# YihanWangAstro/VegasAfterglow

Hardware: AMD Instinct MI355X
Metric: light-curves/sec (single model) and MCMC walker-steps/sec at 1/2/4/8 MI355X (higher is better)
Workload: dtype f64

## Files before the change

vegasafterglow_amd/csrc/vag_capi.hip:

```cpp
#include <hip/hip_runtime.h>

#include <algorithm>
#include <cmath>
#include <cstdarg>
#include <cstdio>
#include <cstdlib>
#include <cstring>
#include <memory>
#include <string>
#include <vector>
#include <atomic>
#include <chrono>
#include <condition_variable>
#include <map>
#include <mutex>
#include <shared_mutex>

#include "vag_ic_kernels.h"
#include "vag_kernels.h"
#include "vag_rs_kernels.h"
#include "vag_fit_rows.h"
#include "vag_grid_rows.h"
#include "vag_sky.h"
#include "vag_debug_math.h"
// ... 537 lines not shown
}

}

static int ctx_init(vag_ctx* c) {
    HIPCHK(hipStreamCreateWithFlags(&c->own_stream, hipStreamNonBlocking));
    c->stream = c->own_stream;
    for (auto& e : c->ev) HIPCHK(hipEventCreate(&e));
    HIPCHK(hipEventCreateWithFlags(&c->ev_handoff, hipEventDisableTiming));
    HIPCHK(hipDeviceGetAttribute(&c->n_cus, hipDeviceAttributeMultiprocessorCount, c->device));
    for (const void* fn : {reinterpret_cast<const void*>(vag_flux_grid_kernel<false, FLUX_SYN>),
                           reinterpret_cast<const void*>(vag_flux_grid_kernel<true, FLUX_SYN>),
                           reinterpret_cast<const void*>(vag_flux_grid_kernel<false, FLUX_SYN_IC>),
                           reinterpret_cast<const void*>(vag_flux_grid_kernel<false, FLUX_SSC>),
                           reinterpret_cast<const void*>(vag_flux_grid_kernel<false, FLUX_SYN, false, 256>),
                           reinterpret_cast<const void*>(vag_flux_grid_kernel<false, FLUX_SYN_IC, false, 256>),
                           reinterpret_cast<const void*>(vag_flux_grid_kernel<false, FLUX_SSC, false, 256>),
                           reinterpret_cast<const void*>(vag_flux_grid_kernel<false, FLUX_SYN, true>),
                           reinterpret_cast<const void*>(vag_flux_grid_kernel<false, FLUX_SYN_IC, true>),
                           reinterpret_cast<const void*>(vag_flux_grid_kernel<false, FLUX_SSC, true>),
                           reinterpret_cast<const void*>(vag_flux_grid_kernel<false, FLUX_FUSED>),
                           reinterpret_cast<const void*>(vag_flux_grid_kernel<false, FLUX_FUSED, false, 256>),
                           reinterpret_cast<const void*>(vag_flux_grid_kernel<false, FLUX_FUSED, true>),
                           reinterpret_cast<const void*>(vag_flux_series_kernel<FLUX_SYN, true>),
                           reinterpret_cast<const void*>(vag_flux_series_kernel<FLUX_SYN_IC, true>),
                           reinterpret_cast<const void*>(vag_flux_series_kernel<FLUX_SSC, true>)})
        HIPCHK(hipFuncSetAttribute(fn, hipFuncAttributeMaxDynamicSharedMemorySize, 160 * 1024));
    {
        std::vector<double> lut(2 * KN_LUT_N);
        const double step = (KN_LG2_XMAX - KN_LG2_XMIN) / (double)(KN_LUT_N - 1);
        for (int i = 0; i < KN_LUT_N; ++i) {
            const double x = std::exp2(KN_LG2_XMIN + step * (double)i);
            double ratio;
            if (x < 1e-2) {
                ratio = 1 - 2 * x;
            } else if (x > 1e2) {
                ratio = 3. / 8 * (std::log(2 * x) + 0.5) / x;
            } else {
                const double l = std::log1p(2.0 * x), invx = 1.0 / x, invx2 = invx * invx;
                const double invt1 = 1.0 / (1.0 + 2.0 * x), invt1_2 = invt1 * invt1;
                ratio = 0.75 * ((1.0 + x) * invx2 * invx * (2.0 * x * (1.0 + x) * invt1 - l) + 0.5 * l * invx -
                                (1.0 + 3.0 * x) * invt1_2);
            }
            lut[i] = ratio;
            lut[KN_LUT_N + i] = std::log2(ratio);
        }
// ... 551 lines not shown
    long long lo = 4;
    if (c->total_pairs / 16 >= 2048) lo = 16;
    if (c->total_pairs / 64 >= 4096) lo = 64;
    ppb = std::max(ppb, lo);
    ppb = std::min<long long>(ppb, std::max(1, c->max_pairs));
    return (int)std::max<long long>(1, ppb);
}

static int flux_ks(const vag_ctx* c) {
    int cap = 512;
    if (const char* e = vag_hook("VAG_FLUX_K_CAP")) cap = std::max(4, std::atoi(e));
    return std::max(2, std::min(c->max_k, cap));
}

static int* work_counters(vag_ctx* c) { return reinterpret_cast<int*>(reinterpret_cast<char*>(c->d_plan.p) + sizeof(VagDevPlan)) + 4; }

static size_t flux_grid_lds_bytes(int mode, int ks, int nt, int nnu) {
    const size_t slots = (size_t)nt * nnu;
    size_t d = (size_t)(VAG_NPAR + 4) * ks + (size_t)ks * nnu + 2 * (size_t)nt + nnu + SP_LDS_DOUBLES + slots;
    if (mode == FLUX_FUSED) d += 6 * (size_t)ks + (size_t)ks * nnu + slots;
    return sizeof(double) * d + sizeof(int) * nt + 16;
}

int run_flux_series(vag_ctx* c, const vag_model_params* d_params, int nb, const double* d_lg2t, const double* d_lg2nu, int n,
                    double* d_out, int mode = FLUX_SYN, int n_bands = 0, int grid_nt = 0);

static void launch_reduce(hipStream_t st, const vag_model_params* d_params, const VagGridMeta* meta, const double* partial, int max_blocks,
                          int ppb, int nt, int nnu, const double* d_bandw, double* d_out, int nb,
                          int* work_counter = nullptr ) {
    if (d_bandw) {
        hipLaunchKernelGGL(vag_reduce_kernel, dim3((nt + 255) / 256, nb), dim3(256), 0, st, d_params, meta, partial, max_blocks, ppb, nt, nnu,
                           d_bandw, d_out, work_counter);
    } else {
        const int slots = nt * nnu;
        hipLaunchKernelGGL(vag_reduce_grid_kernel, dim3((slots + REDUCE_SLOTS - 1) / REDUCE_SLOTS, nb), dim3(REDUCE_GROUPS * REDUCE_SLOTS), 0, st,
                           d_params, meta, partial, max_blocks, ppb, slots, d_out, work_counter);
    }
}

constexpr int FLUX_PERSIST_MIN_PPB = 128;
template <bool COUNT, int MODE, bool SPREAD = false, int THREADS = FLUX_THREADS, bool PIECES = false>
static bool launch_flux_grid(vag_ctx* c, FluxArgs a, int nb, size_t lds, int persist) {
    const auto fn = vag_flux_grid_kernel<COUNT, MODE, SPREAD, THREADS, PIECES, true>;
    int wg = -1;
    if (persist) {
        for (const auto& e : c->flux_occ)
            if (e.fn == reinterpret_cast<const void*>(fn) && e.lds == lds) wg = e.wg;
        if (wg < 0) {
            (void)hipFuncSetAttribute(reinterpret_cast<const void*>(fn), hipFuncAttributeMaxDynamicSharedMemorySize, 160 * 1024);
            if (hipOccupancyMaxActiveBlocksPerMultiprocessor(&wg, fn, THREADS, lds) != hipSuccess || wg < 1) wg = 1;
            if (c->flux_occ.size() > 256) c->flux_occ.clear();
            c->flux_occ.push_back({reinterpret_cast<const void*>(fn), lds, wg});
        }
    }
    if (!persist || (persist == 1 && (a.n_items <= (long long)wg * c->n_cus || a.pairs_per_block < FLUX_PERSIST_MIN_PPB))) {
        if (vag_hook("VAG_DEBUG_LAUNCH")) std::fprintf(stderr, "[vag] grid flux form: one item per workgroup, %d x %d\n", a.max_blocks, nb);
        a.work = nullptr;
        hipLaunchKernelGGL((vag_flux_grid_kernel<COUNT, MODE, SPREAD, THREADS, PIECES>), dim3(a.max_blocks, nb), dim3(THREADS), lds, c->stream, a);
        return false;
    }
    const long long n_wg = std::min<long long>(a.n_items, (long long)wg * c->n_cus);
    if (vag_hook("VAG_DEBUG_LAUNCH"))
        std::fprintf(stderr, "[vag] grid flux form: persistent, %lld workgroups for %d items\n", n_wg, a.n_items);
    hipLaunchKernelGGL(vag_flux_order_kernel, dim3((nb + 3) / 4), dim3(256), 0, c->stream, a.meta, nb, const_cast<int*>(a.order));
    hipLaunchKernelGGL(fn, dim3((unsigned)n_wg), dim3(THREADS), lds, c->stream, a);
    return true;
}

int run_flux_grid(vag_ctx* c, const vag_model_params* d_params, int nb, const double* d_lg2t, int nt,
                  const double* d_lg2nu, int nnu, const double* d_bandw, double* d_out, int mode = FLUX_SYN,
                  double* d_out2 = nullptr ) {
    hipStream_t st = c->stream;
    StageScope ps(c, mode == FLUX_SSC ? PS_SSC_FLUX : PS_SYNC_FLUX);
    const int slots = nt * nnu;
    if (slots <= SERIES_THREADS * SERIES_MAX_SLOTS && nnu <= SERIES_MAX_BANDS && !d_bandw && mode != FLUX_FUSED && !c->count_work &&
        vag_hook("VAG_GRID_ROWWISE") && !(c->batch_flags & VAG_FLAG_SPREADING))
        return run_flux_series(c, d_params, nb, d_lg2t, d_lg2nu, slots, d_out, mode, nnu, nt);
    if (slots > FLUX_MAX_SLOTS)
        return set_err(VAG_E_CAPACITY, "nt*nnu = %d exceeds %d per launch", slots, FLUX_MAX_SLOTS);
    {
        const long long blocks = (c->total_pairs + FITROWS_ROWS - 1) / FITROWS_ROWS;
        if (mode != FLUX_FUSED && !(c->batch_flags & VAG_FLAG_SPREADING) && !c->count_work && slots <= GRIDROWS_MAX_SLOTS &&
            nnu <= GRIDROWS_BANDS && nt <= GRIDROWS_MAX_NT && blocks >= 4096 && c->total_pairs >= 128LL * nb && c->n_rows > 0 &&
            !c->ppb_pin && !vag_hook("VAG_GRID_ROW_PER_WORKGROUP")) {
            const int max_blocks = std::max(1, (c->max_pairs + FITROWS_ROWS - 1) / FITROWS_ROWS);
            if (c->d_partial.ensure(sizeof(double) * (size_t)nb * max_blocks * slots)) return VAG_E_HIP;
            SeriesArgs a{};
            a.params = d_params;
// ... 94 lines not shown
    c->plan.interps += c->total_pairs * (long long)nt * nnu;
    c->plan.flux_blocks = max_blocks * nb;
    c->plan.pairs_per_block = ppb;
    bool persistent = false;
    if (c->n_rows > 0) {
        const bool small = !spreading && !a.work_count && (long long)nt * nnu <= 512 && (long long)ks * ((nnu + 1) / 2) <= 512 &&
                           !vag_hook("VAG_FLUX_WIDE");
        if (vag_hook("VAG_DEBUG_LAUNCH")) {
            int occ = -1;
            if (small && mode == FLUX_SSC)
                (void)hipOccupancyMaxActiveBlocksPerMultiprocessor(&occ, vag_flux_grid_kernel<false, FLUX_SSC, false, 256>, 256, lds);
            else if (small && mode == FLUX_SYN_IC)
                (void)hipOccupancyMaxActiveBlocksPerMultiprocessor(&occ, vag_flux_grid_kernel<false, FLUX_SYN_IC, false, 256>, 256, lds);
            else if (small)
                (void)hipOccupancyMaxActiveBlocksPerMultiprocessor(&occ, vag_flux_grid_kernel<false, FLUX_SYN, false, 256>, 256, lds);
            else if (mode == FLUX_SYN && !spreading)
                (void)hipOccupancyMaxActiveBlocksPerMultiprocessor(&occ, vag_flux_grid_kernel<false, FLUX_SYN>, FLUX_THREADS, lds);
            std::fprintf(stderr, "[vag] grid flux launch: mode %d nt=%d nnu=%d ks=%d rows/wg=%d lanes=%d lds=%zu B wg/CU=%d\n", mode, nt, nnu, ks,
                         ppb, small ? 256 : FLUX_THREADS, lds, occ);
        }
        const bool pieces = c->max_k > ks;
        int persist = 1;
        if (const char* e = vag_hook("VAG_FLUX_PERSISTENT")) persist = std::atoi(e);
        if (persist) {
            if (c->d_flux_order.ensure(sizeof(int) * (size_t)nb)) return VAG_E_HIP;
            a.work = work_counters(c);
            a.order = c->d_flux_order.as<int>();
        }
        if (pieces) {
            a.work_count = nullptr;
#define VAG_PIECES_LAUNCH(M_)                                                                                          \
    do {                                                                                                               \
        if (spreading)                                                                                                 \
            persistent = launch_flux_grid<false, M_, true, FLUX_THREADS, true>(c, a, nb, lds, persist);                         \
        else                                                                                                           \
            persistent = launch_flux_grid<false, M_, false, FLUX_THREADS, true>(c, a, nb, lds, persist);                        \
    } while (0)
            if (mode == FLUX_FUSED)
                VAG_PIECES_LAUNCH(FLUX_FUSED);
            else if (mode == FLUX_SYN_IC)
                VAG_PIECES_LAUNCH(FLUX_SYN_IC);
            else if (mode == FLUX_SSC)
                VAG_PIECES_LAUNCH(FLUX_SSC);
            else
                VAG_PIECES_LAUNCH(FLUX_SYN);
#undef VAG_PIECES_LAUNCH
// ... 1 lines not shown
            persistent = launch_flux_grid<false, FLUX_FUSED, false, 256>(c, a, nb, lds, persist);
        else if (spreading && mode == FLUX_FUSED)
            persistent = launch_flux_grid<false, FLUX_FUSED, true>(c, a, nb, lds, persist);
        else if (mode == FLUX_FUSED)
            persistent = launch_flux_grid<false, FLUX_FUSED>(c, a, nb, lds, persist);
        else if (small && mode == FLUX_SYN_IC)
            persistent = launch_flux_grid<false, FLUX_SYN_IC, false, 256>(c, a, nb, lds, persist);
        else if (small && mode == FLUX_SSC)
            persistent = launch_flux_grid<false, FLUX_SSC, false, 256>(c, a, nb, lds, persist);
        else if (small)
            persistent = launch_flux_grid<false, FLUX_SYN, false, 256>(c, a, nb, lds, persist);
        else if (spreading && mode == FLUX_SYN_IC)
            persistent = launch_flux_grid<false, FLUX_SYN_IC, true>(c, a, nb, lds, persist);
        else if (spreading && mode == FLUX_SSC)
            persistent = launch_flux_grid<false, FLUX_SSC, true>(c, a, nb, lds, persist);
        else if (spreading)
            persistent = launch_flux_grid<false, FLUX_SYN, true>(c, a, nb, lds, persist);
        else if (mode == FLUX_SYN_IC)
            persistent = launch_flux_grid<false, FLUX_SYN_IC>(c, a, nb, lds, persist);
        else if (mode == FLUX_SSC)
            persistent = launch_flux_grid<false, FLUX_SSC>(c, a, nb, lds, persist);
        else if (a.work_count)
            persistent = launch_flux_grid<true, FLUX_SYN>(c, a, nb, lds, persist);
        else
            persistent = launch_flux_grid<false, FLUX_SYN>(c, a, nb, lds, persist);
        HIPCHK(hipGetLastError());
    }
    HIPCHK(hipEventRecord(c->ev[4], st));
    if (a.work_count) {
        unsigned long long h[2];
        HIPCHK(hipMemcpyAsync(h, c->d_workcount.p, sizeof h, hipMemcpyDeviceToHost, st));
        HIPCHK(hipStreamSynchronize(st));
        c->plan.spec_evals += (long long)h[0] - c->eat_cells * nnu;
        c->plan.interps += (long long)h[1] - c->total_pairs * (long long)nt * nnu;
    }
    launch_reduce(st, d_params, c->d_meta.as<VagGridMeta>(), c->d_partial.as<double>(), max_blocks, ppb, nt, nnu, d_bandw, d_out, nb,
                  persistent ? a.work : nullptr);
    if (mode == FLUX_FUSED)
        launch_reduce(st, d_params, c->d_meta.as<VagGridMeta>(), c->d_partial2.as<double>(), max_blocks, ppb, nt, nnu, d_bandw, d_out2, nb);
    HIPCHK(hipGetLastError());
    HIPCHK(hipEventRecord(c->ev[5], st));
    return VAG_OK;
}

__global__ void vag_add_kernel(double* __restrict__ out, const double* __restrict__ add, size_t n) {
    for (size_t i = (size_t)blockIdx.x * blockDim.x + threadIdx.x; i < n; i += (size_t)gridDim.x * blockDim.x) out[i] += add[i];
// ... 3682 lines not shown
```

vegasafterglow_amd/csrc/vag_kernels.h:

```cpp
#pragma once
#include "vag_device.h"
#include "vag_grid_kernel.h"
#include "vag_dyn_fast.h"

namespace vag {

struct Layout {
    const int* row_off;
    const long long* cell_off;
};

VAG_DEV int find_model(const int* off, int nb, int idx) {
    int lo = 0, hi = nb;
    while (hi - lo > 1) {
        const int mid = (lo + hi) >> 1;
        if (off[mid] <= idx)
            lo = mid;
        else
            hi = mid;
    }
    return lo;
}

VAG_DEV int cell_model(const long long* __restrict__ cell_off, int nb, long long c) {
// ... 680 lines not shown
    g.cos_th = __hiloint2double(t[1], t[0]), g.sin_th = __hiloint2double(t[3], t[2]), g.dth = __hiloint2double(t[5], t[4]);
    g.rep = t[6];
    g.cph = __hiloint2double(p[1], p[0]), g.dph = __hiloint2double(p[3], p[2]);
    g.cos_obs = __hiloint2double(h[1], h[0]), g.sin_obs = __hiloint2double(h[3], h[2]);
    return g;
}
#else
struct RowGeo {
    double cos_th, sin_th, dth, cph, dph, cos_obs, sin_obs;
    int rep;
    VAG_DEV double cos_view() const { return fma(cos_th, cos_obs, (sin_th * cph) * sin_obs); }
};
VAG_DEV RowGeo sload_rowgeo(const double* rg, int th_byte, int j, int i) {
    const double* t = rg + th_byte / 8 + 4 * j;
    const double* p = rg + ROWGEO_HDR + 2 * i;
    RowGeo g;
    g.cos_th = t[0], g.sin_th = t[1], g.dth = t[2], g.rep = __double2loint(t[3]);
    g.cph = p[0], g.dph = p[1], g.cos_obs = rg[0], g.sin_obs = rg[1];
    return g;
}
VAG_DEV int sload_i32(const int* p) { return *p; }
#endif

VAG_DEV void eat_row(const double* __restrict__ s_par, int KS, int K, int tid, int nthreads, double cos_v,
                     double t_coeff, double one_plus_z, double lg2_dOmega, double* __restrict__ s_t,
                     double* __restrict__ s_dop, double* __restrict__ s_geom, LdsTab lg, int* win = nullptr, double w_lo = 0,
                     double w_hi = 0) {
    WinCount wc;
    for (int k = tid; k < K; k += nthreads) {
        const double* c = s_par + k * VAG_NPAR;
        const LdsTab c2 = lds_tab(c);
        const vdouble2 Gu = c2[VP_GAMMA / 2], rt = c2[VP_R / 2];
        const double G = Gu.x, u = Gu.y, r = rt.x;
#if defined(VAG_FLUX_ABLATE) && (VAG_FLUX_ABLATE & 8)
        s_dop[k] = G, s_t[k] = 3.0 + 0.1 * k + u, s_geom[k] = r;
        continue;
#endif
        const double lg2_dop = -log2_tab(fma(-u, cos_v, G), lg);
        const double time = fma(t_coeff, r, rt.y * one_plus_z);
        const double lt = log2_tab(time, lg);
        s_dop[k] = lg2_dop;
        s_t[k] = lt;
        s_geom[k] = (lg2_dOmega + c[VP_LG2_R2]) + 3.0 * lg2_dop;
        if (win) wc.add(true, lt, w_lo, w_hi);
    }
    if (win) wc.store(win, tid);
}

VAG_DEV void eat_row_spread(const double* __restrict__ s_par, int KS, int K, int tid, int nthreads,
                            const double* __restrict__ geo, double cos_phi, double sin_obs, double cos_obs, double lg2_dphi,
                            double one_plus_z, double* __restrict__ s_t, double* __restrict__ s_dop,
                            double* __restrict__ s_geom, LdsTab lg, int GS ,
                            int* win = nullptr, double w_lo = 0, double w_hi = 0) {
    WinCount wc;
    for (int k = tid; k < K; k += nthreads) {
        const double* c = s_par + k * VAG_NPAR;
        const LdsTab c2 = lds_tab(c);
        const vdouble2 Gu = c2[VP_GAMMA / 2], rt = c2[VP_R / 2];
        const double G = Gu.x, u = Gu.y, r = rt.x;
        const double cos_v = geo[GS + k] * cos_phi * sin_obs + geo[k] * cos_obs;
        const double lg2_dop = -log2_tab(G - u * cos_v, lg);
        const double time = (rt.y + (1 - cos_v) * r / C_C) * one_plus_z;
        const double lt = log2_tab(time, lg);
        s_dop[k] = lg2_dop;
        s_t[k] = lt;
        s_geom[k] = ((geo[2 * GS + k] + lg2_dphi) + c[VP_LG2_R2]) + 3.0 * lg2_dop;
// ... 25 lines not shown
                       const int* __restrict__ rep_of, const double* __restrict__ cellpar,
                       const double* __restrict__ cell_theta ,
                       double* __restrict__ out_t, double* __restrict__ out_dop) {
    const VagGridMeta M = meta[0];
    if (M.status != 0) return;
    const int K = M.n_t, nth = M.n_theta;
    const long long total = (long long)M.n_phi_eff * nth * K;
    const long long q = (long long)blockIdx.x * blockDim.x + threadIdx.x;
    if (q >= total) return;
    const int k = (int)(q % K), j = (int)((q / K) % nth), i = (int)(q / ((long long)K * nth));
    const vag_model_params P = params[0];
    const double one_plus_z = 1 + P.z;
    const int rep = rep_of[j] + i * M.rep_phi_stride;
    const double* par = cellpar + (long long)rep * K * VAG_NPAR;
    const double G = par[VP_GAMMA * K + k], r = par[VP_R * K + k], teng = par[VP_TENG * K + k];
    const double th = cell_theta ? cell_theta[(long long)rep * K + k] : theta[j];
    const double s_half = sin(0.5 * (th - P.theta_obs)), s_phi = sin(0.5 * phi[i]);
    const double one_minus_cos_v = 2 * s_half * s_half + 2 * sin(th) * sin(P.theta_obs) * (s_phi * s_phi);
    const double u = sqrt((G - 1) * (G + 1));
    out_t[q] = (teng + one_minus_cos_v * r / C_C) * one_plus_z / U_SEC;
    out_dop[q] = 1.0 / (1.0 / (G + u) + u * one_minus_cos_v);
}

template <bool COUNT, int MODE, bool SPREAD, int THREADS, bool PIECES>
__device__ __forceinline__ void flux_grid_item(const FluxArgs& a, const int m, const int blk) {
    const VagGridMeta* Mp = a.meta + m;
    if (Mp->status != 0) return;
    const int n_phi_eff = Mp->n_phi_eff;
    const int n_pairs = Mp->n_theta * n_phi_eff;
    const int p0 = blk * a.pairs_per_block;
    if (p0 >= n_pairs) return;
    const int p1 = min(n_pairs, p0 + a.pairs_per_block);
    const int tid = threadIdx.x;
    const int K_all = Mp->n_t, KS = a.k_stride;
    const int n_pieces = (!PIECES || K_all <= KS) ? 1 : (K_all - 1 + KS - 2) / (KS - 1);
    int K = min(K_all, KS), k0 = 0;
    const int nt = a.nt, nnu = a.nnu;
    const int slots = nt * nnu;

    extern __shared__ __attribute__((aligned(16))) double lds[];
    double* s_sp = lds;
    double* s_par = s_sp + SP_LDS_DOUBLES;
    double* s_t = s_par + VAG_NPAR * KS;
    double* s_dop = s_t + 2 * KS;
    double* s_geom = s_dop + KS;
    double* s_B = s_geom + KS;
// ... 63 lines not shown
#endif
    const double* gth = a.geo_th + (size_t)m * 3 * Mp->th_stride;
    const double* gph = a.geo_ph + (size_t)m * 2 * Mp->ph_stride;
    auto stage_and_eat = [&](int j, int i, int buf) {
        const double w_lo = s_tobs[0], w_hi = s_tobs[nt - 1];
        if constexpr (SPREAD) {
            const double* geo = a.cellgeo + (a.cell_off[m] + (long long)rep_at(j, i) * K_all) * 3 + k0;
            eat_row_spread(s_par, KS, K, etid, THREADS, geo, gph[i], sin_obs, cos_obs, gph[Mp->ph_stride + i], one_plus_z,
                           s_t + buf * KS, s_dop, s_geom, lg_tab, K_all, s_win + buf * 2, w_lo, w_hi);
        } else {
            const RowGeo g = sload_rowgeo(rg, rg_th, j, i);
            const double cos_v = g.cos_view();
            const double t_coeff = (1 - cos_v) * opz_over_c;
            const double lg2_dOmega = g.dth + g.dph;
            eat_row(s_par, KS, K, etid, THREADS, cos_v, t_coeff, one_plus_z, lg2_dOmega, s_t + buf * KS, s_dop, s_geom, lg_tab,
                    s_win + buf * 2, w_lo, w_hi);
        }
    };
    int staged_rep = -1;
    auto stage_row = [&](int j, int i) {
        const int rep = rep_at(j, i);
        if (rep != staged_rep) {
            const double* src = a.cellpar + (a.cell_off[m] + (long long)rep * K_all) * VAG_NPAR + k0;
#pragma unroll 1
            for (int q = tid; q < VAG_NPAR * K; q += THREADS) {
                const int par = (int)(((float)q + 0.5f) / (float)K);
                s_par[(q - par * K) * VAG_NPAR + par] = src[(size_t)par * K_all + (q - par * K)];
            }
            if constexpr (MODE == FLUX_SSC) {
                __syncthreads();
                const double* hdr0 = a.ichdr + (size_t)(a.cell_off[m] + (long long)rep * K_all + k0) * FLUX_IC_HDR;
#pragma unroll 1
                for (int q = tid; q < 6 * K; q += THREADS) {
                    const int kk = q / 6, w = q - kk * 6;
                    s_par[kk * VAG_NPAR + w] = hdr0[(size_t)kk * FLUX_IC_HDR + w];
                }
            }
            if constexpr (MODE == FLUX_FUSED) {
                const double* hdr0 = a.ichdr + (size_t)(a.cell_off[m] + (long long)rep * K_all + k0) * FLUX_IC_HDR;
#pragma unroll 1
                for (int q = tid; q < 6 * K; q += THREADS) {
                    const int kk = q / 6, w = q - kk * 6;
                    s_hdr[kk * 6 + w] = hdr0[(size_t)kk * FLUX_IC_HDR + w];
                }
            }
            staged_rep = rep;
            return true;
        }
        return false;
    };
    for (int piece = 0; piece < n_pieces; ++piece) {
// ... 5 lines not shown
    }
    __syncthreads();
    int jn = p0 / n_phi_eff, in_ = p0 - jn * n_phi_eff;
    stage_row(jn, in_);
    __syncthreads();
    stage_and_eat(jn, in_, 0);
    __syncthreads();
    VAG_FLUX_MARK(7);
    for (int pair = p0; pair < p1; ++pair) {
        const int buf = (pair - p0) & 1;
        if (++in_ == n_phi_eff) in_ = 0, ++jn;
        const double* s_tc = s_t + buf * KS;
        const double row_t0 = s_tc[0], row_tN = s_tc[K - 1];
        for (int idx = tid; idx < nt; idx += THREADS) {
            const double tq = s_tobs[idx];
            int kk = 0;
            double w = NAN;
#if defined(VAG_FLUX_ABLATE) && (VAG_FLUX_ABLATE & 4)
            if (tq >= row_t0 && tq < row_tN) kk = min(idx, K - 2), w = 0.5;
            if (false) {
#else
            if (tq >= row_t0 && tq < row_tN) {
#endif
                int lo = s_kidx[idx], hi;
                lo = min(max(lo, 1), K - 3);
                const double ta = s_tc[lo - 1], tb = s_tc[lo], tc = s_tc[lo + 1], td = s_tc[lo + 2];
                if (K >= 4 && ta <= tq && tq < td) {
                    lo = tq < tb ? lo - 1 : (tq < tc ? lo : lo + 1);
                } else {
                    lo = K >= 4 ? lo : 0;
                    if (s_tc[lo] <= tq) {
                        int step = 1;
                        hi = lo + 1;
                        while (hi < K - 1 && s_tc[hi] <= tq) {
                            lo = hi;
                            step <<= 1;
                            hi = min(lo + step, K - 1);
                        }
                    } else {
                        int step = 1;
                        hi = lo;
                        lo = hi - 1;
                        while (s_tc[lo] > tq) {
                            hi = lo;
                            step <<= 1;
                            lo = max(hi - step, 0);
                        }
                    }
                    while (hi - lo > 1) {
                        const int mid = (lo + hi) >> 1;
                        if (s_tc[mid] <= tq)
                            lo = mid;
                        else
                            hi = mid;
                    }
                }
                kk = lo;
                const double t_lo = s_tc[lo];
                w = (tq - t_lo) * (1.0 / (s_tc[lo + 1] - t_lo));
            }
            s_kidx[idx] = kk;
            s_w[idx] = w;
        }
        VAG_FLUX_MARK(0);
        const double w_lo = s_tobs[0], w_hi = s_tobs[nt - 1];
        const bool in_window = !(row_tN < w_lo || row_t0 > w_hi);
        if (in_window) {
            const int lane = tid & 63;
            int n_lt = 0, n_le = 0;
#if defined(VAG_FLUX_ABLATE) && (VAG_FLUX_ABLATE & 16)
            n_lt = 1, n_le = K;
#else
            n_lt = __builtin_amdgcn_readfirstlane(s_win[buf * 2]);
            n_le = __builtin_amdgcn_readfirstlane(s_win[buf * 2 + 1]);
#endif
            const int k_lo = n_lt > 0 ? n_lt - 1 : 0;
            const int k_hi = min(max(n_le, k_lo + 1), K - 1);
            const int nk = k_hi - k_lo + 1;
            const int npair_nu = (nnu + 1) >> 1;
            const int total = nk * npair_nu;
            const float inv_nk = __builtin_amdgcn_rcpf((float)nk);
            if constexpr (COUNT) {
// ... 102 lines not shown
                }
                int kq[U], iq[U];
                double lo[U], hi[U], wq[U], aq[U];
                [[maybe_unused]] double lo2[U], hi2[U], aq2[U];
#pragma unroll
                for (int u = UB; u < UE; ++u) {
                    iq[u] = dv[u] & 0xffff;
                    kq[u] = s_kidx[iq[u]];
                }
#pragma unroll
                for (int u = UB; u < UE; ++u) {
                    const int kk = ((dv[u] >> 16) & 0x7fff) + kq[u];
                    lo[u] = s_B[kk], hi[u] = s_B[kk + 1];
                    wq[u] = s_w[iq[u]];
                    aq[u] = s_acc[min(slot0 + u * THREADS, slots - 1)];
                    if constexpr (MODE == FLUX_FUSED) {
                        lo2[u] = s_B2[kk], hi2[u] = s_B2[kk + 1];
                        aq2[u] = s_acc2[min(slot0 + u * THREADS, slots - 1)];
                    }
                }
                [[maybe_unused]] bool sp_a = false, sp_b = false;
                [[maybe_unused]] double e_dop = 0, e_lt = 0;
                if constexpr (decltype(with_eat)::value) {
                    e_dop = -log2_tab_core(fma(-e_Gu.y, e_cos, e_Gu.x), lg_tab, sp_a);
                    e_lt = log2_tab_core(fma(e_tc, e_rt.x, e_rt.y * one_plus_z), lg_tab, sp_b);
                }
#pragma unroll
                for (int u = UB; u < UE; ++u) {
                    const double x = fma(hi[u] - lo[u], wq[u], lo[u]);
                    aq[u] += exp2_or_zero(x);
                    if constexpr (MODE == FLUX_FUSED) {
                        const double x2 = fma(hi2[u] - lo2[u], wq[u], lo2[u]);
                        aq2[u] += exp2_or_zero(x2);
                    }
                }
#pragma unroll
                for (int u = UB; u < UE; ++u)
                    if (dv[u] >= 0) {
                        s_acc[slot0 + u * THREADS] = aq[u];
                        if constexpr (MODE == FLUX_FUSED) s_acc2[slot0 + u * THREADS] = aq2[u];
                    }
                if constexpr (decltype(with_eat)::value) {
                    if (sp_a) e_dop = -log2(fma(-e_Gu.y, e_cos, e_Gu.x));
                    if (__builtin_expect(sp_b, 0)) e_lt = log2(fma(e_tc, e_rt.x, e_rt.y * one_plus_z));
                    WinCount wc;
                    wc.add(tid < K, e_lt, w_lo, w_hi);
                    wc.store(s_win + (buf ^ 1) * 2, tid);
                    if (tid < K) {
                        s_dop[ek] = e_dop;
                        s_t[(buf ^ 1) * KS + ek] = e_lt;
                        s_geom[ek] = (e_dom + e_r2) + 3.0 * e_dop;
                    }
                }
            };
#if defined(VAG_FLUX_ABLATE) && (VAG_FLUX_ABLATE & 2)
            if (false)
#endif
            {
                using I0 = std::integral_constant<int, 0>;
                using IH = std::integral_constant<int, U / 2>;
                using IU = std::integral_constant<int, U>;
                if (fuse_eat && (tid & ~63) < K) {
                    interp_group(desc0, tid, std::true_type{}, I0{}, IH{});
                    interp_group(desc0, tid, std::false_type{}, IH{}, IU{});
                } else {
                    interp_group(desc0, tid, std::false_type{}, I0{}, IU{});
                }
                for (int slot0 = tid + U * THREADS; slot0 - tid < slots; slot0 += U * THREADS) {
                    int dq[U];
#pragma unroll
                    for (int u = 0; u < U; ++u) dq[u] = slot_desc(slot0 + u * THREADS);
                    interp_group(dq, slot0, std::false_type{}, I0{}, IU{});
                }
            }
            if (fuse_eat) {
                if (THREADS < 512 && K > THREADS) {
                    const RowGeo g = sload_rowgeo(rg, rg_th, jn, in_);
                    const double cos_v = g.cos_view();
                    const double t_coeff = (1 - cos_v) * opz_over_c;
                    const double lg2_dOmega = g.dth + g.dph;
                    WinCount wc;
                    for (int k = tid + THREADS; k < K; k += THREADS) {
                        const double* c = s_par + k * VAG_NPAR;
                        const LdsTab c2 = lds_tab(c);
                        const vdouble2 Gu = c2[VP_GAMMA / 2], rt = c2[VP_R / 2];
                        const double lg2_dop = -log2_tab(fma(-Gu.y, cos_v, Gu.x), lg_tab);
                        const double lt = log2_tab(fma(t_coeff, rt.x, rt.y * one_plus_z), lg_tab);
                        s_dop[k] = lg2_dop;
                        s_t[(buf ^ 1) * KS + k] = lt;
                        s_geom[k] = (lg2_dOmega + c[VP_LG2_R2]) + 3.0 * lg2_dop;
                        wc.add(true, lt, w_lo, w_hi);
                    }
                    wc.store(s_win + (buf ^ 1) * 2, tid);
                }
            }
        }
        VAG_FLUX_MARK(4);
#ifdef VAG_FLUX_PRIO
        __builtin_amdgcn_s_setprio(0);
#endif
        __syncthreads();
        VAG_FLUX_MARK(5);
        if (__builtin_expect(have_next && !same_rep, 0)) {
            stage_row(jn, in_);
            __syncthreads();
            stage_and_eat(jn, in_, buf ^ 1);
            __syncthreads();
            VAG_FLUX_MARK(6);
        }
    }
    }
#ifdef VAG_FLUX_STAMPS
    if (m == 0 && blk == 1 && (tid & 63) == 0)
// ... 18 lines not shown
    }
}

template <bool COUNT, int MODE, bool SPREAD = false, int THREADS = FLUX_THREADS, bool PIECES = false, bool PERSIST = false>
__global__ void __launch_bounds__(THREADS, 4)
vag_flux_grid_kernel(FluxArgs a) {
    extern __shared__ __attribute__((aligned(16))) double lds[];
    for (int i = threadIdx.x; i < SP_LDS_DOUBLES; i += THREADS) lds[i] = a.sp_table[i];
    if constexpr (!PERSIST) {
        flux_grid_item<COUNT, MODE, SPREAD, THREADS, PIECES>(a, blockIdx.y, blockIdx.x);
        return;
    }
    int* s_it = reinterpret_cast<int*>(lds + SP_LDS_DOUBLES);
    for (;;) {
        __syncthreads();
        if (threadIdx.x == 0) *s_it = __hip_atomic_fetch_add(a.work, 1, __ATOMIC_RELAXED, __HIP_MEMORY_SCOPE_AGENT);
        __syncthreads();
        const int it = __builtin_amdgcn_readfirstlane(*s_it);
        if (it >= a.n_items) break;
        const int r = it / a.max_blocks;
        flux_grid_item<COUNT, MODE, SPREAD, THREADS, PIECES>(a, a.order[r], it - r * a.max_blocks);
    }
}

__global__ void __launch_bounds__(256)
vag_flux_order_kernel(const VagGridMeta* __restrict__ meta, int nb, int* __restrict__ order) {
    auto cost = [&](int j) -> long long {
        const VagGridMeta& M = meta[j];
        return M.status == 0 ? (long long)M.n_theta * M.n_phi_eff * M.n_t : -1;
    };
    const int m = blockIdx.x * 4 + (threadIdx.x >> 6), lane = threadIdx.x & 63;
    if (m >= nb) return;
    const long long c = cost(m);
    int ahead = 0;
#pragma unroll 4
    for (int j = lane; j < nb; j += 64) {
        const long long d = cost(j);
        ahead += d > c || (d == c && j < m);
    }
#pragma unroll
    for (int o = 32; o > 0; o >>= 1) ahead += __shfl_xor(ahead, o);
    if (lane == 0) order[ahead] = m;
}

__global__ void __launch_bounds__(256)
vag_reduce_kernel(const vag_model_params* __restrict__ params, const VagGridMeta* __restrict__ meta,
// ... 452 lines not shown
```

Measured before the change: 25110.

## Add warp-specialised split flux kernel overlapping boundary spectra with interpolation

Adds a persistent flux-grid kernel that splits each workgroup into two wavefront teams. One team computes the EAT step and the per-frequency boundary spectra for the next row into double-buffered LDS, while the other team interpolates and accumulates the current row with per-thread register accumulators. The goal is to overlap spectrum evaluation with interpolation and cut repeated LDS reads. It is enabled by default only for the synchronous path with exactly 10 frequencies, enough times and large K, and falls back otherwise. Shared helpers are factored out of the existing kernel without changing behaviour. Costs are more registers and barriers, plus a risk of load imbalance between the two teams.

```diff
diff --git a/vegasafterglow_amd/csrc/vag_capi.hip b/vegasafterglow_amd/csrc/vag_capi.hip
--- a/vegasafterglow_amd/csrc/vag_capi.hip
+++ b/vegasafterglow_amd/csrc/vag_capi.hip
@@ -583,6 +583,7 @@
                            reinterpret_cast<const void*>(vag_flux_grid_kernel<false, FLUX_FUSED>),
                            reinterpret_cast<const void*>(vag_flux_grid_kernel<false, FLUX_FUSED, false, 256>),
                            reinterpret_cast<const void*>(vag_flux_grid_kernel<false, FLUX_FUSED, true>),
+                           reinterpret_cast<const void*>(vag_flux_grid_split_kernel),
                            reinterpret_cast<const void*>(vag_flux_series_kernel<FLUX_SYN, true>),
                            reinterpret_cast<const void*>(vag_flux_series_kernel<FLUX_SYN_IC, true>),
                            reinterpret_cast<const void*>(vag_flux_series_kernel<FLUX_SSC, true>)})
@@ -1180,6 +1181,9 @@
     return sizeof(double) * d + sizeof(int) * nt + 16;
 }
 
+constexpr size_t FLUX_SPLIT_LDS_BUDGET = 81920;
+static size_t flux_split_lds_bytes(int ks, int nt, int nnu) { return FluxSplitLds(ks, nt, nnu).bytes; }
+
 int run_flux_series(vag_ctx* c, const vag_model_params* d_params, int nb, const double* d_lg2t, const double* d_lg2nu, int n,
                     double* d_out, int mode = FLUX_SYN, int n_bands = 0, int grid_nt = 0);
 
@@ -1197,6 +1201,7 @@
 }
 
 constexpr int FLUX_PERSIST_MIN_PPB = 128;
+constexpr int FLUX_SPLIT_MIN_KS = 192;
 template <bool COUNT, int MODE, bool SPREAD = false, int THREADS = FLUX_THREADS, bool PIECES = false>
 static bool launch_flux_grid(vag_ctx* c, FluxArgs a, int nb, size_t lds, int persist) {
     const auto fn = vag_flux_grid_kernel<COUNT, MODE, SPREAD, THREADS, PIECES, true>;
@@ -1222,6 +1227,32 @@
         std::fprintf(stderr, "[vag] grid flux form: persistent, %lld workgroups for %d items\n", n_wg, a.n_items);
     hipLaunchKernelGGL(vag_flux_order_kernel, dim3((nb + 3) / 4), dim3(256), 0, c->stream, a.meta, nb, const_cast<int*>(a.order));
     hipLaunchKernelGGL(fn, dim3((unsigned)n_wg), dim3(THREADS), lds, c->stream, a);
+    return true;
+}
+
+static bool launch_flux_grid_split(vag_ctx* c, FluxArgs a, int nb, int persist, int split) {
+    if (!split || !persist || !a.rowgeo) return false;
+    const size_t lds = flux_split_lds_bytes(a.k_stride, a.nt, a.nnu);
+    if (lds > FLUX_SPLIT_LDS_BUDGET || a.nnu > FLUX_SPLIT_MAX_NNU || a.nt > FLUX_SPLIT_MAX_NT) return false;
+    if (split == 1 && (a.nnu != FLUX_SPLIT_MAX_NNU || a.nt <= FLUX_SPLIT_B * 64 || a.k_stride < FLUX_SPLIT_MIN_KS)) return false;
+    const auto fn = vag_flux_grid_split_kernel;
+    int wg = -1;
+    for (const auto& e : c->flux_occ)
+        if (e.fn == reinterpret_cast<const void*>(fn) && e.lds == lds) wg = e.wg;
+    if (wg < 0) {
+        if (hipOccupancyMaxActiveBlocksPerMultiprocessor(&wg, fn, FLUX_THREADS, lds) != hipSuccess || wg < 1) wg = 1;
+        if (c->flux_occ.size() > 256) c->flux_occ.clear();
+        c->flux_occ.push_back({reinterpret_cast<const void*>(fn), lds, wg});
+    }
+    if (persist == 1 && (a.n_items <= (long long)wg * c->n_cus || a.pairs_per_block < FLUX_PERSIST_MIN_PPB)) return false;
+    const long long n_wg = std::min<long long>(a.n_items, (long long)wg * c->n_cus);
+    if (vag_hook("VAG_DEBUG_LAUNCH")) {
+        std::fprintf(stderr, "[vag] grid flux form: persistent, %lld workgroups for %d items\n", n_wg, a.n_items);
+        std::fprintf(stderr, "[vag] grid flux split: %d + %d wavefronts (boundary spectra + interpolation), lds=%zu B wg/CU=%d\n", FLUX_SPLIT_A,
+                     FLUX_SPLIT_B, lds, wg);
+    }
+    hipLaunchKernelGGL(vag_flux_order_kernel, dim3((nb + 3) / 4), dim3(256), 0, c->stream, a.meta, nb, const_cast<int*>(a.order));
+    hipLaunchKernelGGL(fn, dim3((unsigned)n_wg), dim3(FLUX_THREADS), lds, c->stream, a);
     return true;
 }
 
@@ -1362,6 +1393,8 @@
         const bool pieces = c->max_k > ks;
         int persist = 1;
         if (const char* e = vag_hook("VAG_FLUX_PERSISTENT")) persist = std::atoi(e);
+        int split = 1;
+        if (const char* e = vag_hook("VAG_FLUX_SPLIT")) split = std::atoi(e);
         if (persist) {
             if (c->d_flux_order.ensure(sizeof(int) * (size_t)nb)) return VAG_E_HIP;
             a.work = work_counters(c);
@@ -1409,6 +1442,8 @@
             persistent = launch_flux_grid<false, FLUX_SSC>(c, a, nb, lds, persist);
         else if (a.work_count)
             persistent = launch_flux_grid<true, FLUX_SYN>(c, a, nb, lds, persist);
+        else if (launch_flux_grid_split(c, a, nb, persist, split))
+            persistent = true;
         else
             persistent = launch_flux_grid<false, FLUX_SYN>(c, a, nb, lds, persist);
         HIPCHK(hipGetLastError());
diff --git a/vegasafterglow_amd/csrc/vag_kernels.h b/vegasafterglow_amd/csrc/vag_kernels.h
--- a/vegasafterglow_amd/csrc/vag_kernels.h
+++ b/vegasafterglow_amd/csrc/vag_kernels.h
@@ -726,6 +726,10 @@
 VAG_DEV int sload_i32(const int* p) { return *p; }
 #endif
 
+VAG_DEV double eat_doppler_arg(vdouble2 Gu, double cos_v) { return fma(-Gu.y, cos_v, Gu.x); }
+VAG_DEV double eat_time_arg(vdouble2 rt, double t_coeff, double one_plus_z) { return fma(t_coeff, rt.x, rt.y * one_plus_z); }
+VAG_DEV double eat_geom(double lg2_dOmega, double lg2_r2, double lg2_dop) { return (lg2_dOmega + lg2_r2) + 3.0 * lg2_dop; }
+
 VAG_DEV void eat_row(const double* __restrict__ s_par, int KS, int K, int tid, int nthreads, double cos_v,
                      double t_coeff, double one_plus_z, double lg2_dOmega, double* __restrict__ s_t,
                      double* __restrict__ s_dop, double* __restrict__ s_geom, LdsTab lg, int* win = nullptr, double w_lo = 0,
@@ -740,12 +744,12 @@
         s_dop[k] = G, s_t[k] = 3.0 + 0.1 * k + u, s_geom[k] = r;
         continue;
 #endif
-        const double lg2_dop = -log2_tab(fma(-u, cos_v, G), lg);
-        const double time = fma(t_coeff, r, rt.y * one_plus_z);
+        const double lg2_dop = -log2_tab(eat_doppler_arg(Gu, cos_v), lg);
+        const double time = eat_time_arg(rt, t_coeff, one_plus_z);
         const double lt = log2_tab(time, lg);
         s_dop[k] = lg2_dop;
         s_t[k] = lt;
-        s_geom[k] = (lg2_dOmega + c[VP_LG2_R2]) + 3.0 * lg2_dop;
+        s_geom[k] = eat_geom(lg2_dOmega, c[VP_LG2_R2], lg2_dop);
         if (win) wc.add(true, lt, w_lo, w_hi);
     }
     if (win) wc.store(win, tid);
@@ -817,6 +821,53 @@
     out_dop[q] = 1.0 / (1.0 / (G + u) + u * one_minus_cos_v);
 }
 
+VAG_DEV void stage_photon_block(double* __restrict__ s_par, const double* __restrict__ src, int K, int K_all, int tid, int nthreads) {
+#pragma unroll 1
+    for (int q = tid; q < VAG_NPAR * K; q += nthreads) {
+        const int par = (int)(((float)q + 0.5f) / (float)K);
+        s_par[(q - par * K) * VAG_NPAR + par] = src[(size_t)par * K_all + (q - par * K)];
+    }
+}
+
+VAG_DEV void flux_bracket(const double* __restrict__ s_tc, int K, double tq, const int* hint, int& kk, double& w) {
+    int lo = *hint, hi;
+    lo = min(max(lo, 1), K - 3);
+    const double ta = s_tc[lo - 1], tb = s_tc[lo], tc = s_tc[lo + 1], td = s_tc[lo + 2];
+    if (K >= 4 && ta <= tq && tq < td) {
+        lo = tq < tb ? lo - 1 : (tq < tc ? lo : lo + 1);
+    } else {
+        lo = K >= 4 ? lo : 0;
+        if (s_tc[lo] <= tq) {
+            int step = 1;
+            hi = lo + 1;
+            while (hi < K - 1 && s_tc[hi] <= tq) {
+                lo = hi;
+                step <<= 1;
+                hi = min(lo + step, K - 1);
+            }
+        } else {
+            int step = 1;
+            hi = lo;
+            lo = hi - 1;
+            while (s_tc[lo] > tq) {
+                hi = lo;
+                step <<= 1;
+                lo = max(hi - step, 0);
+            }
+        }
+        while (hi - lo > 1) {
+            const int mid = (lo + hi) >> 1;
+            if (s_tc[mid] <= tq)
+                lo = mid;
+            else
+                hi = mid;
+        }
+    }
+    kk = lo;
+    const double t_lo = s_tc[lo];
+    w = (tq - t_lo) * (1.0 / (s_tc[lo + 1] - t_lo));
+}
+
 template <bool COUNT, int MODE, bool SPREAD, int THREADS, bool PIECES>
 __device__ __forceinline__ void flux_grid_item(const FluxArgs& a, const int m, const int blk) {
     const VagGridMeta* Mp = a.meta + m;
@@ -926,11 +977,7 @@
         const int rep = rep_at(j, i);
         if (rep != staged_rep) {
             const double* src = a.cellpar + (a.cell_off[m] + (long long)rep * K_all) * VAG_NPAR + k0;
-#pragma unroll 1
-            for (int q = tid; q < VAG_NPAR * K; q += THREADS) {
-                const int par = (int)(((float)q + 0.5f) / (float)K);
-                s_par[(q - par * K) * VAG_NPAR + par] = src[(size_t)par * K_all + (q - par * K)];
-            }
+            stage_photon_block(s_par, src, K, K_all, tid, THREADS);
             if constexpr (MODE == FLUX_SSC) {
                 __syncthreads();
                 const double* hdr0 = a.ichdr + (size_t)(a.cell_off[m] + (long long)rep * K_all + k0) * FLUX_IC_HDR;
@@ -982,42 +1029,7 @@
 #else
             if (tq >= row_t0 && tq < row_tN) {
 #endif
-                int lo = s_kidx[idx], hi;
-                lo = min(max(lo, 1), K - 3);
-                const double ta = s_tc[lo - 1], tb = s_tc[lo], tc = s_tc[lo + 1], td = s_tc[lo + 2];
-                if (K >= 4 && ta <= tq && tq < td) {
-                    lo = tq < tb ? lo - 1 : (tq < tc ? lo : lo + 1);
-                } else {
-                    lo = K >= 4 ? lo : 0;
-                    if (s_tc[lo] <= tq) {
-                        int step = 1;
-                        hi = lo + 1;
-                        while (hi < K - 1 && s_tc[hi] <= tq) {
-                            lo = hi;
-                            step <<= 1;
-                            hi = min(lo + step, K - 1);
-                        }
-                    } else {
-                        int step = 1;
-                        hi = lo;
-                        lo = hi - 1;
-                        while (s_tc[lo] > tq) {
-                            hi = lo;
-                            step <<= 1;
-                            lo = max(hi - step, 0);
-                        }
-                    }
-                    while (hi - lo > 1) {
-                        const int mid = (lo + hi) >> 1;
-                        if (s_tc[mid] <= tq)
-                            lo = mid;
-                        else
-                            hi = mid;
-                    }
-                }
-                kk = lo;
-                const double t_lo = s_tc[lo];
-                w = (tq - t_lo) * (1.0 / (s_tc[lo + 1] - t_lo));
+                flux_bracket(s_tc, K, tq, s_kidx + idx, kk, w);
             }
             s_kidx[idx] = kk;
             s_w[idx] = w;
@@ -1166,8 +1178,8 @@
                 [[maybe_unused]] bool sp_a = false, sp_b = false;
                 [[maybe_unused]] double e_dop = 0, e_lt = 0;
                 if constexpr (decltype(with_eat)::value) {
-                    e_dop = -log2_tab_core(fma(-e_Gu.y, e_cos, e_Gu.x), lg_tab, sp_a);
-                    e_lt = log2_tab_core(fma(e_tc, e_rt.x, e_rt.y * one_plus_z), lg_tab, sp_b);
+                    e_dop = -log2_tab_core(eat_doppler_arg(e_Gu, e_cos), lg_tab, sp_a);
+                    e_lt = log2_tab_core(eat_time_arg(e_rt, e_tc, one_plus_z), lg_tab, sp_b);
                 }
 #pragma unroll
                 for (int u = UB; u < UE; ++u) {
@@ -1185,15 +1197,15 @@
                         if constexpr (MODE == FLUX_FUSED) s_acc2[slot0 + u * THREADS] = aq2[u];
                     }
                 if constexpr (decltype(with_eat)::value) {
-                    if (sp_a) e_dop = -log2(fma(-e_Gu.y, e_cos, e_Gu.x));
-                    if (__builtin_expect(sp_b, 0)) e_lt = log2(fma(e_tc, e_rt.x, e_rt.y * one_plus_z));
+                    if (sp_a) e_dop = -log2(eat_doppler_arg(e_Gu, e_cos));
+                    if (__builtin_expect(sp_b, 0)) e_lt = log2(eat_time_arg(e_rt, e_tc, one_plus_z));
                     WinCount wc;
                     wc.add(tid < K, e_lt, w_lo, w_hi);
                     wc.store(s_win + (buf ^ 1) * 2, tid);
                     if (tid < K) {
                         s_dop[ek] = e_dop;
                         s_t[(buf ^ 1) * KS + ek] = e_lt;
-                        s_geom[ek] = (e_dom + e_r2) + 3.0 * e_dop;
+                        s_geom[ek] = eat_geom(e_dom, e_r2, e_dop);
                     }
                 }
             };
@@ -1228,11 +1240,11 @@
                         const double* c = s_par + k * VAG_NPAR;
                         const LdsTab c2 = lds_tab(c);
                         const vdouble2 Gu = c2[VP_GAMMA / 2], rt = c2[VP_R / 2];
-                        const double lg2_dop = -log2_tab(fma(-Gu.y, cos_v, Gu.x), lg_tab);
-                        const double lt = log2_tab(fma(t_coeff, rt.x, rt.y * one_plus_z), lg_tab);
+                        const double lg2_dop = -log2_tab(eat_doppler_arg(Gu, cos_v), lg_tab);
+                        const double lt = log2_tab(eat_time_arg(rt, t_coeff, one_plus_z), lg_tab);
                         s_dop[k] = lg2_dop;
                         s_t[(buf ^ 1) * KS + k] = lt;
-                        s_geom[k] = (lg2_dOmega + c[VP_LG2_R2]) + 3.0 * lg2_dop;
+                        s_geom[k] = eat_geom(lg2_dOmega, c[VP_LG2_R2], lg2_dop);
                         wc.add(true, lt, w_lo, w_hi);
                     }
                     wc.store(s_win + (buf ^ 1) * 2, tid);
@@ -1297,6 +1309,277 @@
         flux_grid_item<COUNT, MODE, SPREAD, THREADS, PIECES>(a, a.order[r], it - r * a.max_blocks);
     }
 }
+
+#ifndef VAG_HOST_DEBUG
+constexpr int FLUX_SPLIT_A = 6;
+constexpr int FLUX_SPLIT_B = FLUX_THREADS / 64 - FLUX_SPLIT_A;
+constexpr int FLUX_SPLIT_TIMES = 2;
+constexpr int FLUX_SPLIT_MAX_NT = FLUX_SPLIT_TIMES * FLUX_SPLIT_B * 64;
+constexpr int FLUX_SPLIT_MAX_NNU = 10;
+constexpr int FLUX_SPLIT_E = 2;
+constexpr int FLUX_SPLIT_E0 = FLUX_SPLIT_A - FLUX_SPLIT_E;
+constexpr int FLUX_SPLIT_GROUP = 5;
+static_assert(FLUX_SPLIT_A >= FLUX_SPLIT_E && FLUX_SPLIT_B >= 1, "both teams need wavefronts, the A team those of the EAT step");
+static_assert(FLUX_SPLIT_MAX_NNU % FLUX_SPLIT_GROUP == 0, "the full set of frequencies is taken in whole groups");
+
+struct FluxSplitLds {
+    int par, t, dop, B, tobs, nu, win;
+    size_t bytes;
+    __host__ __device__ FluxSplitLds(int ks, int nt, int nnu) {
+        par = SP_LDS_DOUBLES;
+        t = par + VAG_NPAR * ks;
+        dop = t + 3 * ks;
+        B = dop + 2 * ks;
+        tobs = B + 2 * nnu * ks;
+        nu = tobs + nt;
+        win = nu + nnu;
+        bytes = sizeof(double) * (size_t)win + sizeof(int) * 4 * FLUX_SPLIT_E;
+    }
+};
+
+__device__ __forceinline__ void flux_split_item(const FluxArgs& a, const int m, const int blk) {
+    constexpr int THREADS = FLUX_THREADS, NB = FLUX_SPLIT_B, AL = FLUX_SPLIT_A * 64, BL = NB * 64, NE = FLUX_SPLIT_E, EL = NE * 64;
+    const VagGridMeta* Mp = a.meta + m;
+    if (Mp->status != 0) return;
+    const int n_phi_eff = Mp->n_phi_eff;
+    const int n_pairs = Mp->n_theta * n_phi_eff;
+    const int p0 = blk * a.pairs_per_block;
+    if (p0 >= n_pairs) return;
+    const int n_rows = min(n_pairs, p0 + a.pairs_per_block) - p0;
+    const int tid = threadIdx.x;
+    const int K = Mp->n_t, KS = a.k_stride;
+    const int nt = a.nt, nnu = a.nnu;
+
+    extern __shared__ __attribute__((aligned(16))) double lds[];
+    const FluxSplitLds L(KS, nt, nnu);
+    double* s_sp = lds;
+    double* s_par = lds + L.par;
+    double* s_t = lds + L.t;
+    double* s_dop = lds + L.dop;
+    double* s_B = lds + L.B;
+    double* s_tobs = lds + L.tobs;
+    double* s_nu = lds + L.nu;
+    int* s_win = reinterpret_cast<int*>(lds + L.win);
+
+    const vag_model_params* Pp = a.params + m;
+    const double one_plus_z = 1 + Pp->z;
+    const double opz_over_c = one_plus_z / C_C;
+    {
+        const double lg2_1pz = Mp->lg2_1pz;
+        for (int i = tid; i < nt; i += THREADS) s_tobs[i] = a.lg2_t_obs[i];
+        for (int l = tid; l < nnu; l += THREADS) s_nu[l] = a.lg2_nu_obs[l] + lg2_1pz;
+    }
+    SpecConst sc;
+    sc.init(Pp->p);
+    const double* rg = a.rowgeo + (size_t)m * a.rowgeo_stride;
+    const int rg_th = sload_i32(reinterpret_cast<const int*>(rg + 2));
+    auto rep_at = [&](int j) { return sload_i32(reinterpret_cast<const int*>(reinterpret_cast<const char*>(rg) + rg_th + 32 * j + 24)); };
+    const LdsTab sp_tab = lds_tab(s_sp), lg_tab = lds_tab(s_sp + SP_TABLE_DOUBLES);
+    const int wave = __builtin_amdgcn_readfirstlane(tid >> 6);
+    const bool a_team = wave < FLUX_SPLIT_A;
+    const int lane = tid & 63;
+
+    auto stage = [&](int rep) {
+        const double* src = a.cellpar + (a.cell_off[m] + (long long)rep * K) * VAG_NPAR;
+        stage_photon_block(s_par, src, K, K, tid, THREADS);
+    };
+    auto pipeline = [&](auto&& work, auto&& late_eat) {
+        int j1 = p0 / n_phi_eff, i1 = p0 - j1 * n_phi_eff;
+        int staged_rep = rep_at(j1);
+        __syncthreads();
+        stage(staged_rep);
+        __syncthreads();
+        late_eat(j1, i1, 0, 0);
+        __syncthreads();
+        int tb0 = 2, tb1 = 0, tb2 = 1;
+        for (int n = -1; n < n_rows; ++n) {
+            int j2 = j1, i2 = i1 + 1;
+            if (i2 == n_phi_eff) i2 = 0, ++j2;
+            const bool have2 = n + 2 < n_rows;
+            const int rep2 = have2 ? rep_at(j2) : staged_rep;
+            const bool same = rep2 == staged_rep;
+            work(n, j1, i1, j2, i2, tb0, tb1, tb2, have2 && same);
+            __syncthreads();
+            if (__builtin_expect(!same, 0)) {
+                stage(rep2);
+                staged_rep = rep2;
+                __syncthreads();
+                late_eat(j2, i2, n + 2, tb2);
+                __syncthreads();
+            }
+            j1 = j2, i1 = i2;
+            tb0 = tb1, tb1 = tb2, tb2 = tb2 == 2 ? 0 : tb2 + 1;
+        }
+    };
+
+    auto eat = [&](int j, int i, int r, int tb) {
+        const int etid = tid - FLUX_SPLIT_E0 * 64, ew = wave - FLUX_SPLIT_E0;
+        if (ew < 0) return;
+        const double w_lo = s_tobs[0], w_hi = s_tobs[nt - 1];
+        const RowGeo g = sload_rowgeo(rg, rg_th, j, i);
+        const double cos_v = g.cos_view();
+        const double t_coeff = (1 - cos_v) * opz_over_c;
+        double* st = s_t + tb * KS;
+        double* sd = s_dop + (r & 1) * KS;
+        int n_lt = 0, n_le = 0;
+        for (int k = etid; k < K; k += EL) {
+            const LdsTab c2 = lds_tab(s_par + k * VAG_NPAR);
+            const vdouble2 Gu = c2[VP_GAMMA / 2], rt = c2[VP_R / 2];
+            bool sp_a, sp_b;
+            double dop = -log2_tab_core(eat_doppler_arg(Gu, cos_v), lg_tab, sp_a);
+            double lt = log2_tab_core(eat_time_arg(rt, t_coeff, one_plus_z), lg_tab, sp_b);
+            if (__builtin_expect(sp_a, 0)) dop = -log2(eat_doppler_arg(Gu, cos_v));
+            if (__builtin_expect(sp_b, 0)) lt = log2(eat_time_arg(rt, t_coeff, one_plus_z));
+            sd[k] = dop;
+            st[k] = lt;
+            n_lt += __popcll(__ballot(lt < w_lo));
+            n_le += __popcll(__ballot(lt <= w_hi));
+        }
+        if (lane == 0) {
+            int* win = s_win + ((r & 1) * NE + ew) * 2;
+            win[0] = n_lt, win[1] = n_le;
+        }
+    };
+    if (a_team) {
+        const int atid = tid;
+        auto spectra_of = [&](int n, int j1, int i1, int tb1) {
+            const int r = n + 1;
+            if (r >= n_rows) return;
+            const double* s_tc = s_t + tb1 * KS;
+            const double row_t0 = s_tc[0], row_tN = s_tc[K - 1];
+            const double w_lo = s_tobs[0], w_hi = s_tobs[nt - 1];
+            if (row_tN < w_lo || row_t0 > w_hi) return;
+            const int* win = s_win + (r & 1) * 2 * NE;
+            int n_lt = 0, n_le = 0;
+#pragma unroll
+            for (int w = 0; w < NE; ++w) {
+                n_lt += __builtin_amdgcn_readfirstlane(win[2 * w]);
+                n_le += __builtin_amdgcn_readfirstlane(win[2 * w + 1]);
+            }
+            const int k_lo = n_lt > 0 ? n_lt - 1 : 0;
+            const int k_hi = min(max(n_le, k_lo + 1), K - 1);
+            const RowGeo g = sload_rowgeo(rg, rg_th, j1, i1);
+            const double lg2_dOmega = g.dth + g.dph;
+            const double* dopv = s_dop + (r & 1) * KS;
+            double* sB = s_B + (r & 1) * nnu * KS;
+            const int nk = k_hi - k_lo + 1;
+            const int total = nk * ((nnu + 1) >> 1);
+            const float inv_nk = __builtin_amdgcn_rcpf((float)nk);
+            const int dq_l = AL / nk, dq_k = AL - dq_l * nk;
+            int lg = (int)(((float)atid + 0.5f) * inv_nk);
+            int kk = atid - __mul24(lg, nk);
+            int bofs = __mul24(lg, 2 * KS);
+            const int top = (nnu - 1) * KS;
+            for (int q = atid; q < total; q += AL) {
+                const int k = k_lo + kk;
+                const int l0 = lg * 2, l1 = min(l0 + 1, nnu - 1);
+                const double dop = dopv[k];
+                const SpecRegs regs = load_spec_regs(lds_tab(s_par) + __mul24(k, VAG_NPAR / 2));
+                const double geom = eat_geom(lg2_dOmega, regs[VP_LG2_R2], dop);
+                const double b0 = log2_I_nu_fast(regs, 1, sc, s_nu[l0] - dop, sp_tab);
+                const double b1 = log2_I_nu_fast(regs, 1, sc, s_nu[l1] - dop, sp_tab);
+                sB[bofs + k] = b0 + geom;
+                sB[min(bofs + KS, top) + k] = b1 + geom;
+                kk += dq_k;
+                lg += dq_l;
+                bofs += dq_l * 2 * KS;
+                if (kk >= nk) {
+                    kk -= nk;
+                    ++lg;
+                    bofs += 2 * KS;
+                }
+            }
+        };
+        auto spectra = [&](int n, int j1, int i1, int j2, int i2, int, int tb1, int tb2, bool eat_now) {
+            spectra_of(n, j1, i1, tb1);
+            if (eat_now) eat(j2, i2, n + 2, tb2);
+        };
+        pipeline(spectra, eat);
+    } else {
+        const int btid = tid - AL;
+        const double w_lo = a.lg2_t_obs[0], w_hi = a.lg2_t_obs[nt - 1];
+        double acc[FLUX_SPLIT_TIMES][FLUX_SPLIT_MAX_NNU];
+        int hint[FLUX_SPLIT_TIMES];
+        double tq[FLUX_SPLIT_TIMES];
+#pragma unroll
+        for (int o = 0; o < FLUX_SPLIT_TIMES; ++o) {
+            hint[o] = 0;
+            tq[o] = a.lg2_t_obs[min(btid + o * BL, nt - 1)];
+#pragma unroll
+            for (int l = 0; l < FLUX_SPLIT_MAX_NNU; ++l) acc[o][l] = 0;
+        }
+        auto interp = [&](int n, int, int, int, int, int tb0, int, int, bool) {
+            if (n >= 0) {
+                const double* s_tc = s_t + tb0 * KS;
+                const double row_t0 = s_tc[0], row_tN = s_tc[K - 1];
+                if (row_tN < w_lo || row_t0 > w_hi) {
+#pragma unroll
+                    for (int o = 0; o < FLUX_SPLIT_TIMES; ++o) hint[o] = 0;
+                } else {
+                    const double* sB = s_B + (n & 1) * nnu * KS;
+#pragma unroll
+                    for (int o = 0; o < FLUX_SPLIT_TIMES; ++o) {
+                        const bool owned = btid + o * BL < nt;
+                        const bool inside = owned && tq[o] >= row_t0 && tq[o] < row_tN;
+                        int kk = 0;
+                        double w = NAN;
+                        if (inside) flux_bracket(s_tc, K, tq[o], &hint[o], kk, w);
+                        hint[o] = kk;
+                        if (inside) {
+                            if (nnu == FLUX_SPLIT_MAX_NNU) {
+#pragma unroll
+                                for (int l0 = 0; l0 < FLUX_SPLIT_MAX_NNU; l0 += FLUX_SPLIT_GROUP) {
+                                    double lo[FLUX_SPLIT_GROUP], hi[FLUX_SPLIT_GROUP];
+#pragma unroll
+                                    for (int g = 0; g < FLUX_SPLIT_GROUP; ++g) lo[g] = sB[(l0 + g) * KS + kk], hi[g] = sB[(l0 + g) * KS + kk + 1];
+#pragma unroll
+                                    for (int g = 0; g < FLUX_SPLIT_GROUP; ++g) acc[o][l0 + g] += exp2_or_zero(fma(hi[g] - lo[g], w, lo[g]));
+                                    __builtin_amdgcn_sched_barrier(0);
+                                }
+                            } else {
+#pragma unroll
+                                for (int l = 0; l < FLUX_SPLIT_MAX_NNU; ++l) {
+                                    if (l < nnu) {
+                                        const double lo = sB[l * KS + kk], hi = sB[l * KS + kk + 1];
+                                        acc[o][l] += exp2_or_zero(fma(hi - lo, w, lo));
+                                    }
+                                }
+                            }
+                        }
+                    }
+                }
+            }
+        };
+        pipeline(interp, [](int, int, int, int) {});
+        double* my_partial = a.partial + ((size_t)m * a.max_blocks + blk) * ((size_t)nt * nnu);
+#pragma unroll
+        for (int o = 0; o < FLUX_SPLIT_TIMES; ++o) {
+            const int idx = btid + o * BL;
+            if (idx < nt) {
+#pragma unroll
+                for (int l = 0; l < FLUX_SPLIT_MAX_NNU; ++l)
+                    if (l < nnu) my_partial[l * nt + idx] = acc[o][l];
+            }
+        }
+    }
+}
+
+__global__ void __launch_bounds__(FLUX_THREADS, 4)
+vag_flux_grid_split_kernel(FluxArgs a) {
+    extern __shared__ __attribute__((aligned(16))) double lds[];
+    for (int i = threadIdx.x; i < SP_LDS_DOUBLES; i += FLUX_THREADS) lds[i] = a.sp_table[i];
+    int* s_it = reinterpret_cast<int*>(lds + SP_LDS_DOUBLES);
+    for (;;) {
+        __syncthreads();
+        if (threadIdx.x == 0) *s_it = __hip_atomic_fetch_add(a.work, 1, __ATOMIC_RELAXED, __HIP_MEMORY_SCOPE_AGENT);
+        __syncthreads();
+        const int it = __builtin_amdgcn_readfirstlane(*s_it);
+        if (it >= a.n_items) break;
+        const int r = it / a.max_blocks;
+        flux_split_item(a, a.order[r], it - r * a.max_blocks);
+    }
+}
+#endif
 
 __global__ void __launch_bounds__(256)
 vag_flux_order_kernel(const VagGridMeta* __restrict__ meta, int nb, int* __restrict__ order) {
```

Result: faster. 27150, median of 6 (+8.1%).
